# ZechangSun/QFA

Measured on AMD Instinct MI355X. Metric: spectra/sec per EM step, higher is better.
Workload: dtype f32

## Files before the change

### qfa_amd/csrc/qfa_grads_t.h

```cpp
#pragma once
#include "qfa_common.h"
#include "qfa_xdl_kernels.h"
#include "qfa_gt_layout.h"

struct GtPlan {
    int T16, PB, R, gpr;
    int nxcd;
    __host__ __device__ int per_xcd() const { return (PB * R + nxcd - 1) / nxcd; }
    __host__ __device__ int items() const { return nxcd * per_xcd(); }
};

template <int KP>
__device__ __forceinline__ void prep_pgt_body(int bid, const float *__restrict__ F, const float *__restrict__ Psi,
                                              const float *__restrict__ omega, const ZPSrc &ZP, int Npix, int Nb, int Nh,
                                              unsigned char *__restrict__ PGT) {
    using GT = GTT<KP>;
    unsigned char *tile = PGT + (size_t)bid * GT::TILE_B;
    const int p0 = GT::PXW * (bid / GT::TPW) + bid % GT::TPW;
    auto pixel = [&](int lo) { return p0 + GT::TPW * lo; };
    __shared__ float f[16][KP + 1];
    __shared__ float tsc[16][3];
    for (int i = threadIdx.x; i < 16 * KP; i += 256) {
        const int px = i / KP, a = i % KP;
        f[px][a] = (pixel(px) < Npix && a < Nh) ? F[(size_t)pixel(px) * Nh + a] : 0.f;
    }
    __syncthreads();
    if (threadIdx.x < 16) {
        float mx = 0.f;
        for (int a = 0; a < KP; ++a) mx = fmaxf(mx, fabsf(f[threadIdx.x][a]));
        int e = 7;
        if (mx > 0.f && mx < 3.0e38f) (void)frexpf(mx, &e);
        e = e < -50 ? -50 : (e > 60 ? 60 : e);
        tsc[threadIdx.x][0] = ldexpf(1.f, 7 - e);
        tsc[threadIdx.x][1] = ldexpf(1.f, 2 * (e - 7));
        tsc[threadIdx.x][2] = ldexpf(1.f, e - 7);
    }
    __syncthreads();
    for (int i = threadIdx.x; i < GT::NKQ * 64; i += 256) {
        const int lane = i & 63, ks = i >> 6;
        const int px = lane & 15, g = lane >> 4;
        const float t1 = tsc[px][0], t2 = t1 * t1;
        float v[8];
#pragma unroll
        for (int j = 0; j < 8; ++j) {
            const int q = 32 * ks + 8 * g + j;
            float x = 0.f;
            if (q < GT::KK2) {
                int a = 0;
                while (a + 1 < KP && pair_index(a + 1, a + 1, KP) <= q) ++a;
                const int b = a + (q - pair_index(a, a, KP));
                x = f[px][a] * f[px][b] * t2;
            } else {
                const int a = q - (32 * (GT::NKQ - 1) + GT::YOFF);
                if (a >= 0 && a < KP) x = f[px][a] * t1;
            }
            v[j] = x;
        }
        unsigned char *dst = tile + ks * GT::BLK_B + lane * 16;
        u32x4 ph, pm;
        split8h(v, ph, pm);
        *reinterpret_cast<u32x4 *>(dst) = ph;
        *reinterpret_cast<u32x4 *>(dst + 1024) = pm;
    }
    if (threadIdx.x < 128) {
        const int j = threadIdx.x, px = pixel(j & 15);
        float v = 0.f;
        if (j < 16) v = px < Npix ? Psi[px] : 0.f;
        else if (j < 32) v = px < Nb ? omega[px] : 0.f;
        else if (j < 80 && ZP.on() && px < Nb) {
            const float4 q = ZP.at(px);
            v = j < 48 ? q.x : (j < 64 ? q.y : q.z);
        } else if (j >= GT::PAR_IT2 && j < GT::PAR_SBETA) v = tsc[j & 15][j < GT::PAR_IT1 ? 1 : 2];
        else if (j >= GT::PAR_SBETA) v = f16_weight_scale(px < Npix ? Psi[px] : 1.f);
        reinterpret_cast<float *>(tile + GT::OFF_PAR)[j] = v;
    }
    float *fr = reinterpret_cast<float *>(tile + GT::OFF_F);
    for (int i = threadIdx.x; i < 16 * KP; i += 256) fr[i] = f[i / KP][i % KP];
}

#ifndef QFA_GT_STAMPS
#define QFA_GT_STAMPS 0
#endif
#if QFA_GT_STAMPS
__device__ unsigned long long qfa_gt_stamps[2 * 16];
#define GTS(i)                                                                                 \
    {                                                                                          \
        __builtin_amdgcn_sched_barrier(0);                                                     \
        unsigned long long t_;                                                                 \
        asm volatile("s_memtime %0\n\ts_waitcnt lgkmcnt(0)" : "=s"(t_)::"memory");             \
        st_[i] += (unsigned)(t_ - st_last);                                                    \
        st_last = t_;                                                                          \
        __builtin_amdgcn_sched_barrier(0);                                                     \
    }
#else
#define GTS(i) {}
#endif
template <int KP, bool HASA, bool ZF, bool IDX, bool EXACT>
__global__ __launch_bounds__(512, 2) void k_grads_t(qfa_params_t p, qfa_batch_t bt, qfa_tau_t tau, int B, int Npix, int Nb,
                                                    int Nh, GtPlan gp, const unsigned char *__restrict__ PGT,
                                                    const unsigned char *__restrict__ PST, const float4 *__restrict__ ZS,
                                                    float *__restrict__ accum,
                                                    float *__restrict__ slab, double *__restrict__ slabS, int slab_stride,
                                                    Scal64 *__restrict__ sc64) {
    using GT = GTT<KP>;
    __shared__ __attribute__((aligned(16))) unsigned char lds[GT::L_TOTAL];
    const int tid = threadIdx.x;
    const int lane = tid & 63;
    const int wv8 = wave_uniform(tid >> 6);
    const int lo = lane & 15, g = lane >> 4;
    const int item = ((int)blockIdx.x % gp.nxcd) * gp.per_xcd() + ((int)blockIdx.x / gp.nxcd);
    const bool idle = item >= gp.PB * gp.R;
    const int rr = idle ? 0 : item / gp.PB, pb = idle ? 0 : item % gp.PB;
    const int G = (B + 15) >> 4;
    const int g0 = rr * gp.gpr;
    const int n = idle ? 0 : max(0, min(gp.gpr, G - g0));
    constexpr int TPW = GT::TPW, PXW = GT::PXW;
    const int wt = pb + gp.PB * wv8;
#ifndef QFA_GT_ONLY
#define QFA_GT_ONLY 0
#endif
    const bool active = !idle && wt < gp.T16 && (QFA_GT_ONLY == 0 || (QFA_GT_ONLY == 1) == (wv8 < 4));
    int px[TPW];
    bool inb[TPW], blue[TPW];
#pragma unroll
    for (int j = 0; j < TPW; ++j) {
        px[j] = PXW * wt + TPW * lo + j;
        inb[j] = active && px[j] < Npix;
        blue[j] = active && px[j] < Nb;
    }
    const bool blueTile = active && PXW * wt < Nb;
    const DevConsts k = load_consts(p, tau);
    const bool det = slab != nullptr;
    float *accF = det ? slab + (size_t)rr * (size_t)slab_stride : accum;
    float *accA = accF + (size_t)Npix * Nh;
    float *accS = accum + (size_t)Npix * Nh + 3 * (size_t)Npix + Nb;

#if QFA_GT_STAMPS
    unsigned st_[8];
    for (int i = 0; i < 8; ++i) st_[i] = 0;
    unsigned long long st_last;
    asm volatile("s_memtime %0\n\ts_waitcnt lgkmcnt(0)" : "=s"(st_last)::"memory");
#endif
    const unsigned char *tile[TPW];
    u32x4 IBh[TPW][GT::NKQ], IBm[TPW][GT::NKQ];
    float Psi[TPW], om[TPW], ti[TPW], pwi[TPW], l2i[TPW], offl[TPW];
    float it2[TPW], it1[TPW];
    float sbeta[TPW];
    f32x4 zfac = {1.f, 1.f, 1.f, 1.f};
#pragma unroll
    for (int j = 0; j < TPW; ++j) {
        tile[j] = PGT + (size_t)(active ? TPW * wt + j : 0) * GT::TILE_B;
#pragma unroll
        for (int ks = 0; ks < GT::NKQ; ++ks) {
            IBh[j][ks] = *reinterpret_cast<const u32x4 *>(tile[j] + ks * GT::BLK_B + lane * 16);
            IBm[j][ks] = *reinterpret_cast<const u32x4 *>(tile[j] + ks * GT::BLK_B + 1024 + lane * 16);
        }
        const float *par = reinterpret_cast<const float *>(tile[j] + GT::OFF_PAR);
        Psi[j] = par[lo]; om[j] = par[16 + lo];
        it2[j] = par[GT::PAR_IT2 + lo]; it1[j] = par[GT::PAR_IT1 + lo];
        sbeta[j] = par[GT::PAR_SBETA + lo];
        ti[j] = ZF ? par[32 + lo] : 0.f; pwi[j] = ZF ? par[48 + lo] : 0.f; l2i[j] = ZF ? par[64 + lo] : 0.f;
        offl[j] = blue[j] ? k.offp : 0.f;
    }

#pragma unroll
    for (int j = 0; j < TPW; ++j) {
#pragma unroll
        for (int ks = 0; ks < GT::NKQ; ++ks) {
            asm volatile("" ::"v"(IBh[j][ks]), "v"(IBm[j][ks]));
        }
        asm volatile("" ::"v"(Psi[j]), "v"(om[j]), "v"(ti[j]), "v"(pwi[j]), "v"(l2i[j]), "v"(it2[j]), "v"(it1[j]), "v"(sbeta[j]));
    }
    asm volatile("" ::"v"(k.tau0), "v"(k.c0), "v"(k.beta), "v"(k.t_amp), "v"(k.t_lscale), "v"(k.t_expo), "v"(k.t_off), "v"(k.offp),
                 "v"(k.k1), "v"(k.omc0));

    f32x4 W[TPW][GT::NWT], gacc[TPW];
    float gPsi[TPW], gOm[TPW], sA[TPW];
    int cnt[TPW];
    f32x4 betaR[TPW], gamR[TPW];
#pragma unroll
    for (int j = 0; j < TPW; ++j) {
#pragma unroll
        for (int a = 0; a < GT::NWT; ++a) W[j][a] = f32x4{0.f, 0.f, 0.f, 0.f};
        gacc[j] = betaR[j] = gamR[j] = f32x4{0.f, 0.f, 0.f, 0.f};
        gPsi[j] = gOm[j] = sA[j] = 0.f;
        cnt[j] = 0;
    }
    double d_tau0 = 0.0, d_c0 = 0.0, d_beta = 0.0;

    unsigned char *stg = lds + GT::L_STG + wv8 * 2 * GT::STG_B;
    const bool fastp = active && PXW * wt + PXW - 1 < Npix;
    const bool zblue = !ZF && blueTile;
    const bool fastz = !zblue || PXW * wt + PXW - 1 < Nb;
    const bool slow = active && !fastp;
    const bool zstrad = active && fastp && !fastz;
    const bool zfb = ZF && blueTile;
    auto mask_start = [&](int h, int pc) __attribute__((always_inline)) {
        const int st = PXW * wt + 16 * h + 4 * pc;
        return slow ? max(0, min(st, Npix - 4)) : st;
    };
    const unsigned RS = (unsigned)bt.row_stride;
    constexpr bool idx = IDX;
    auto row_index = [&](int t, int bufi, unsigned row, auto first_tag) __attribute__((always_inline)) -> unsigned {
        constexpr bool FIRST = decltype(first_tag)::value;
        const unsigned s0 = 16u * (unsigned)(g0 + t);
        if (!idx) return s0 + row;
        if (FIRST || QFA_TRACKED_LOADS) return (unsigned)bt.rows[s0 + row];
        return (unsigned)reinterpret_cast<const int *>(stg + bufi * GT::STG_B + GT::STG_ROWS)[row];
    };
    struct RowIdx {
        unsigned r[TPW], m;
    };
    auto read_rows = [&](int t, int bufi, auto first_tag) __attribute__((always_inline)) {
        RowIdx ri;
        const int last_row = min(15, B - 1 - 16 * (g0 + t));
        auto slot_row = [&](int q) __attribute__((always_inline)) { return (unsigned)min(q ^ ((q >> 2) & 1), last_row); };
        ri.m = row_index(t, bufi, slot_row(lane >> 2), first_tag);
        if constexpr (TPW == 1) ri.r[0] = ri.m;
        else {
#pragma unroll
            for (int i = 0; i < TPW; ++i) ri.r[i] = row_index(t, bufi, slot_row((64 / (4 * TPW)) * i + lane / (4 * TPW)), first_tag);
        }
        return ri;
    };
    constexpr bool RUNP = !IDX && TPW == 1 && !QFA_TRACKED_LOADS;
    struct SpecRun {
        const unsigned char *d, *e, *z, *m;
    } sr{nullptr, nullptr, nullptr, nullptr};
    unsigned sr_vo = 0u, sr_vz = 0u, sr_om = 0u;
    const bool runok = RUNP && active && !slow && !zstrad;
    if (RUNP) {
        const size_t r2 = (size_t)16 * (size_t)(g0 + 2);
        const unsigned q = (unsigned)lane >> 2, row = q ^ ((q >> 2) & 1u), pc = 16u * (unsigned)wt + 4u * ((unsigned)lane & 3u);
        sr.d = uniform_ptr(reinterpret_cast<const unsigned char *>(bt.delta + r2 * RS));
        sr.e = uniform_ptr(reinterpret_cast<const unsigned char *>(bt.error + r2 * RS) - GT::STG_ARR);
        sr.m = uniform_ptr(reinterpret_cast<const unsigned char *>(bt.mask + r2 * RS) - GT::STG_MASK);
        sr.z = zblue ? uniform_ptr(reinterpret_cast<const unsigned char *>(bt.zabs + r2 * (size_t)Nb) - 2 * GT::STG_ARR)
                     : (zfb ? uniform_ptr(reinterpret_cast<const unsigned char *>(ZS + r2) - 2 * GT::STG_ARR) : sr.d);
        sr_om = row * RS + pc;
        sr_vo = 4u * sr_om;
        sr_vz = zblue ? 4u * (row * (unsigned)Nb + pc) : 16u * ((unsigned)lane & 15u);
    }
    auto stage_req = [&](int bufi, int k) __attribute__((always_inline)) {
        if (k == 0) {
            const unsigned dst = wave_uniform(lds_addr(stg + bufi * GT::STG_B));
            asm volatile("s_mov_b32 m0, %2\n\ts_nop 0\n\tglobal_load_lds_dwordx4 %0, %1" ::"v"(sr_vo), "s"(sr.d), "s"(dst) : "memory");
        } else if (k == 1) asm volatile("global_load_lds_dwordx4 %0, %1 offset:1024" ::"v"(sr_vo), "s"(sr.e) : "memory");
        else if (k == 2) asm volatile("global_load_lds_dwordx4 %0, %1 offset:2048" ::"v"(sr_vz), "s"(sr.z) : "memory");
        else asm volatile("global_load_lds_dword %0, %1 offset:3072" ::"v"(sr_om), "s"(sr.m) : "memory");
    };
    const size_t sr_zinc = zblue ? (size_t)64 * (size_t)(unsigned)Nb : (zfb ? (size_t)256 : (size_t)0);
    auto advance_run = [&]() __attribute__((always_inline)) {
        if (!RUNP) return;
        sr.d += (size_t)64 * RS;
        sr.e += (size_t)64 * RS;
        sr.m += (size_t)16 * RS;
        sr.z += sr_zinc;
    };
    auto stage_spectra = [&](int t, int bufi, const RowIdx &ri, auto first_tag) __attribute__((always_inline)) {
        if (!active) return;
        const int s0 = 16 * (g0 + t);
        const int last_row = min(15, B - 1 - s0);
        const unsigned dst = wave_uniform(lds_addr(stg + bufi * GT::STG_B));
        auto slot_row = [&](int q) __attribute__((always_inline)) { return (unsigned)min(q ^ ((q >> 2) & 1), last_row); };
        auto Rof = [&](unsigned row) __attribute__((always_inline)) -> unsigned { return row_index(t, bufi, row, first_tag); };
#if QFA_TRACKED_LOADS
        {
            float *sf = reinterpret_cast<float *>(stg + bufi * GT::STG_B);
            unsigned char *mb = stg + bufi * GT::STG_B + GT::STG_MASK;
#pragma unroll
            for (int i = 0; i < 4 * TPW; ++i) {
                const int e = 64 * i + lane, q = e / PXW, pl = e % PXW;
                const unsigned R = Rof(slot_row(q));
                const int pxx = PXW * wt + pl;
                const unsigned long long o = (unsigned long long)R * RS + (unsigned)min(pxx, Npix - 1);
                sf[0 * (GT::STG_ARR / 4) + q * PXW + pl] = bt.delta[o];
                sf[1 * (GT::STG_ARR / 4) + q * PXW + pl] = bt.error[o];
                if (zblue) sf[2 * (GT::STG_ARR / 4) + q * PXW + pl] = bt.zabs[(unsigned long long)R * (unsigned)Nb + (unsigned)min(pxx, Nb - 1)];
                mb[(pl >> 4) * 256 + q * 16 + (pl & 15)] = pxx < Npix ? bt.mask[o] : (unsigned char)0;
            }
            if (zfb && lane < 16) reinterpret_cast<float4 *>(sf + 2 * (GT::STG_ARR / 4))[lane] = ZS[s0 + min(lane, last_row)];
            (void)dst;
            return;
        }
#endif
        [&]() __attribute__((always_inline)) {
        const unsigned Rm = ri.m;
        if constexpr (!IDX) {
            if (!slow && !zstrad) {
                const float *dbase = uniform_ptr(bt.delta + (size_t)s0 * RS);
                const float *ebase = uniform_ptr(bt.error + (size_t)s0 * RS);
                const uint8_t *mbase = uniform_ptr(bt.mask + (size_t)s0 * RS);
                const float *zbase = zblue ? uniform_ptr(bt.zabs + (size_t)s0 * Nb) : dbase;
                if (zfb && lane < 16) glds16a(uniform_ptr(ZS + s0), 16u * (unsigned)min(lane, last_row), dst + 2 * GT::STG_ARR);
                if constexpr (TPW == 1) {
                    const unsigned row = slot_row(lane >> 2);
                    const unsigned pc = 16u * (unsigned)wt + 4u * (unsigned)(lane & 3);
                    const unsigned o = row * RS + pc;
                    const unsigned vo = 4u * o, vz = 4u * (row * (unsigned)Nb + pc);
                    const unsigned char *eb = reinterpret_cast<const unsigned char *>(ebase) - GT::STG_ARR;
                    const unsigned char *zb = reinterpret_cast<const unsigned char *>(zbase) - 2 * GT::STG_ARR;
                    const unsigned char *mb_ = reinterpret_cast<const unsigned char *>(mbase) - GT::STG_MASK;
                    if (zblue)
                        asm volatile("s_mov_b32 m0, %7\n\ts_nop 0\n\tglobal_load_lds_dwordx4 %0, %3\n\t"
                                     "global_load_lds_dwordx4 %0, %4 offset:1024\n\tglobal_load_lds_dwordx4 %1, %5 offset:2048\n\t"
                                     "global_load_lds_dword %2, %6 offset:3072"
                                     ::"v"(vo), "v"(vz), "v"(o), "s"(dbase), "s"(eb), "s"(zb), "s"(mb_), "s"(dst) : "memory");
                    else
                        asm volatile("s_mov_b32 m0, %5\n\ts_nop 0\n\tglobal_load_lds_dwordx4 %0, %2\n\t"
                                     "global_load_lds_dwordx4 %0, %3 offset:1024\n\tglobal_load_lds_dword %1, %4 offset:3072"
                                     ::"v"(vo), "v"(o), "s"(dbase), "s"(eb), "s"(mb_), "s"(dst) : "memory");
                } else {
                    constexpr int LPR = 4 * TPW, SPI = 64 / LPR;
#pragma unroll
                    for (int h = 0; h < TPW; ++h)
                        glds4a(mbase, slot_row(lane >> 2) * RS + (unsigned)mask_start(h, lane & 3), dst + GT::STG_MASK + h * 256);
#pragma unroll
                    for (int i = 0; i < TPW; ++i) {
                        const unsigned row = slot_row(SPI * i + lane / LPR);
                        const unsigned pc = (unsigned)(PXW * wt) + 4u * (unsigned)(lane % LPR);
                        glds16a(dbase, 4u * (row * RS + pc), dst + i * 1024);
                        glds16a(ebase, 4u * (row * RS + pc), dst + GT::STG_ARR + i * 1024);
                        if (zblue) glds16a(zbase, 4u * (row * (unsigned)Nb + pc), dst + 2 * GT::STG_ARR + i * 1024);
                    }
                }
                return;
            }
        }
        if (!slow) {
            if constexpr (TPW == 1) {
                const unsigned R = ri.r[0];
                unsigned pc = 16u * (unsigned)wt + 4u * (unsigned)(lane & 3);
                asm volatile("" : "+v"(pc));
                const unsigned long long o = (unsigned long long)R * RS + pc;
                if (zfb && lane < 16) glds16a(uniform_ptr(ZS + s0), 16u * (unsigned)min(lane, last_row), dst + 2 * GT::STG_ARR);
                if (zstrad) {
#pragma unroll 1
                    for (int i = 0; i < 4; ++i) {
                        int pz = min(16 * wt + lo, Nb - 1);
                        asm volatile("" : "+v"(pz));
                        glds4p(lane_ptr<2>(bt.zabs, (unsigned long long)Rof(slot_row(4 * i + g)) * (unsigned)Nb + (unsigned)pz), dst + 2 * GT::STG_ARR + i * 256);
                    }
                }
                const unsigned char *pd = lane_ptr<2>(bt.delta, o);
                const unsigned char *pe = lane_ptr<2>(reinterpret_cast<const unsigned char *>(bt.error) - GT::STG_ARR, o);
                const unsigned char *pm = lane_ptr<0>(bt.mask - GT::STG_MASK, o);
                if (zblue && !zstrad) {
                    const unsigned char *pz = lane_ptr<2>(reinterpret_cast<const unsigned char *>(bt.zabs) - 2 * GT::STG_ARR, (unsigned long long)R * (unsigned)Nb + pc);
                    asm volatile("s_mov_b32 m0, %4\n\ts_nop 0\n\tglobal_load_lds_dwordx4 %0, off\n\t"
                                 "global_load_lds_dwordx4 %1, off offset:1024\n\tglobal_load_lds_dwordx4 %2, off offset:2048\n\t"
                                 "global_load_lds_dword %3, off offset:3072"
                                 ::"v"(pd), "v"(pe), "v"(pz), "v"(pm), "s"(dst) : "memory");
                } else
                    asm volatile("s_mov_b32 m0, %3\n\ts_nop 0\n\tglobal_load_lds_dwordx4 %0, off\n\t"
                                 "global_load_lds_dwordx4 %1, off offset:1024\n\tglobal_load_lds_dword %2, off offset:3072"
                                 ::"v"(pd), "v"(pe), "v"(pm), "s"(dst) : "memory");
            } else {
                constexpr int LPR = 4 * TPW;
                if (zfb && lane < 16) glds16a(uniform_ptr(ZS + s0), 16u * (unsigned)min(lane, last_row), dst + 2 * GT::STG_ARR);
#pragma unroll
                for (int h = 0; h < TPW; ++h) {
                    unsigned ms = (unsigned)mask_start(h, lane & 3);
                    asm volatile("" : "+v"(ms));
                    glds4p(lane_ptr<0>(bt.mask, (unsigned long long)Rm * RS + ms), dst + GT::STG_MASK + h * 256);
                }
#pragma unroll
                for (int i = 0; i < TPW; ++i) {
                    unsigned pc = (unsigned)(PXW * wt) + 4u * (unsigned)(lane % LPR);
                    asm volatile("" : "+v"(pc));
                    const unsigned long long o = (unsigned long long)ri.r[i] * RS + pc;
                    glds16p(lane_ptr<2>(bt.delta, o), dst + i * 1024);
                    glds16p(lane_ptr<2>(bt.error, o), dst + GT::STG_ARR + i * 1024);
                    if (zblue && !zstrad) glds16p(lane_ptr<2>(bt.zabs, (unsigned long long)ri.r[i] * (unsigned)Nb + pc), dst + 2 * GT::STG_ARR + i * 1024);
                }
                if (zstrad) {
#pragma unroll 1
                    for (int i = 0; i < 4 * TPW; ++i) {
                        const int e = 64 * i + lane;
                        int pz = min(PXW * wt + e % PXW, Nb - 1);
                        asm volatile("" : "+v"(pz));
                        glds4p(lane_ptr<2>(bt.zabs, (unsigned long long)Rof(slot_row(e / PXW)) * (unsigned)Nb + (unsigned)pz), dst + 2 * GT::STG_ARR + i * 256);
                    }
                }
            }
            return;
        }
        if (zfb && lane < 16) glds16a(uniform_ptr(ZS + s0), 16u * (unsigned)min(lane, last_row), dst + 2 * GT::STG_ARR);
#pragma unroll 1
        for (int h = 0; h < TPW; ++h) {
            unsigned ms = (unsigned)mask_start(h, lane & 3);
            asm volatile("" : "+v"(ms));
            glds4p(lane_ptr<0>(bt.mask, (unsigned long long)Rm * RS + ms), dst + GT::STG_MASK + h * 256);
        }
#pragma unroll 1
        for (int i = 0; i < 4 * TPW; ++i) {
            const int e = 64 * i + lane, pl = e % PXW;
            const unsigned R = Rof(slot_row(e / PXW));
            int pxx = PXW * wt + pl;
            asm volatile("" : "+v"(pxx));
            const unsigned long long o = (unsigned long long)R * RS + (unsigned)min(pxx, Npix - 1);
            glds4p(lane_ptr<2>(bt.delta, o), dst + i * 256);
            glds4p(lane_ptr<2>(bt.error, o), dst + GT::STG_ARR + i * 256);
            if (zblue) glds4p(lane_ptr<2>(bt.zabs, (unsigned long long)R * (unsigned)Nb + (unsigned)min(pxx, Nb - 1)), dst + 2 * GT::STG_ARR + i * 256);
        }
        }();
        if (idx) {
            const int t2 = min(t + 2, n - 1), s2 = 16 * (g0 + t2);
            if (lane < 16) glds4a(uniform_ptr(bt.rows + s2), 4u * (unsigned)min(lane, B - 1 - s2), dst + GT::STG_ROWS);
        }
    };
    int mask_pos[TPW];
#pragma unroll
    for (int j = 0; j < TPW; ++j) {
        const int pl = TPW * lo + j, h = pl >> 4, pi = pl & 15;
        mask_pos[j] = h * 256 + ((slow && !QFA_TRACKED_LOADS) ? 4 * (pi >> 2) + min(3, PXW * wt + pl - mask_start(h, pi >> 2)) : pi);
    }

    int nduty = 0, drank = 0;
    bool duty = true;
    {
        int nd = 0, rk = 0;
#pragma unroll
        for (int w = 0; w < GT::NW; ++w) {
            const int tw = pb + gp.PB * w;
            const bool d = !(tw < gp.T16 && PXW * tw < Nb);
            if (w < wv8 && d) ++rk;
            if (d) ++nd;
        }
        if (nd >= 5) { nduty = nd; drank = rk; duty = !blueTile; }
        else { nduty = GT::NW; drank = wv8; duty = true; }
    }
    const int s1_q = GT::S1_PCS / nduty, s1_r = GT::S1_PCS % nduty, z_q = GT::Z_PCS / nduty, z_r = GT::Z_PCS % nduty;
    const int s1_first = drank * s1_q + min(drank, s1_r), z_first = drank * z_q + min(drank, z_r);
    const int s1_req = duty ? s1_q + (drank < s1_r ? 1 : 0) : 0, z_req = duty ? z_q + (drank < z_r ? 1 : 0) : 0;
    auto issue_S1 = [&](int t) __attribute__((always_inline)) {
        const unsigned char *src = uniform_ptr(PST + (size_t)(g0 + t) * GT::STATE_B + s1_first * 1024);
        const unsigned dst = wave_uniform(lds_addr(lds + GT::L_S1 + (t & 1) * GT::S1P_B + s1_first * 1024));
        for (int j = 0; j < s1_req; ++j) glds16a(src + 1024 * j, (unsigned)lane * 16u, dst + 1024 * j);
    };
    auto issue_Z = [&](int t) __attribute__((always_inline)) {
        const unsigned char *src = uniform_ptr(PST + (size_t)(g0 + t) * GT::STATE_B + GT::S1P_B + z_first * 1024);
        const unsigned dst = wave_uniform(lds_addr(lds + GT::L_Z + (t & 1) * GT::ZP_B + z_first * 1024));
        for (int j = 0; j < z_req; ++j) glds16a(src + 1024 * j, (unsigned)lane * 16u, dst + 1024 * j);
    };

    struct Part {
        const unsigned char *src;
        unsigned dst;
        int cnt;
    };
    struct NoPart {};
    constexpr unsigned PBIAS = QFA_TRACKED_LOADS ? 0u : 4096u;
    const unsigned lane16 = (unsigned)lane * 16u;
    auto part_begin = [&](const auto &pt) __attribute__((always_inline)) {
        if constexpr (std::is_same_v<std::decay_t<decltype(pt)>, Part>) {
#if !QFA_TRACKED_LOADS
            asm volatile("s_mov_b32 m0, %0\n\ts_nop 0" ::"s"(pt.dst));
#endif
        }
    };
    auto piece = [&](const auto &pt, int j) __attribute__((always_inline)) {
        if constexpr (std::is_same_v<std::decay_t<decltype(pt)>, Part>) {
            if (j < pt.cnt) {
#if QFA_TRACKED_LOADS
                glds16a(pt.src + 1024 * j, lane16, pt.dst + 1024 * j);
#else
#define QFA_PC(J) case J: asm volatile("global_load_lds_dwordx4 %0, %1 offset:%2" ::"v"(lane16), "s"(pt.src), "n"(1024 * J - 4096)); break;
                switch (j) { QFA_PC(0) QFA_PC(1) QFA_PC(2) QFA_PC(3) QFA_PC(4) QFA_PC(5) QFA_PC(6) QFA_PC(7) default: break; }
#undef QFA_PC
#endif
            }
        }
    };
    static_assert((GT::Z_PCS + 4) / 5 <= 8 && (GT::S1_PCS + 4) / 5 <= 8, "a wave's run of a part: at most eight pieces (immediate offsets)");

    f32x4 afy[TPW], aq[TPW];
#pragma unroll
    for (int j = 0; j < TPW; ++j) afy[j] = aq[j] = f32x4{0.f, 0.f, 0.f, 0.f};
    auto stage1 = [&](int t, const auto &pt) __attribute__((always_inline)) {
        __builtin_amdgcn_s_setprio(2);
        part_begin(pt);
        const unsigned char *sp = lds + GT::L_S1 + (t & 1) * GT::S1P_B + lane * 16;
#pragma unroll
        for (int j = 0; j < TPW; ++j) afy[j] = aq[j] = f32x4{0.f, 0.f, 0.f, 0.f};
        constexpr int NP = GT::S1NP;
        u32x4 aop[2][NP];
#pragma unroll
        for (int pc = 0; pc < NP; ++pc) aop[0][pc] = *reinterpret_cast<const u32x4 *>(sp + pc * 1024);
        f32x4 isc[2] = {f32x4{1.f, 1.f, 1.f, 1.f}, f32x4{1.f, 1.f, 1.f, 1.f}};
        const unsigned char *sq = lds + GT::L_S1 + (t & 1) * GT::S1P_B + GT::S1_SCALES + 32 * g;
        isc[0] = *reinterpret_cast<const f32x4 *>(sq);
        isc[1] = *reinterpret_cast<const f32x4 *>(sq + 16);
        zfac = *reinterpret_cast<const f32x4 *>(lds + GT::L_S1 + (t & 1) * GT::S1P_B + GT::S1_ZFAC + 16 * g);
#pragma unroll
        for (int ks = 0; ks < GT::NKS; ++ks) {
            if (ks + 1 < GT::NKS) {
#pragma unroll
                for (int pc = 0; pc < NP; ++pc)
                    aop[(ks + 1) & 1][pc] = *reinterpret_cast<const u32x4 *>(sp + (ks + 1) * GT::BLK_B + pc * 1024);
            }
            piece(pt, ks);
            if (ks == GT::NKS - 1) piece(pt, GT::NKS);
            const u32x4 &ah = aop[ks & 1][0], &am = aop[ks & 1][1];
#pragma unroll
            for (int j = 0; j < TPW; ++j) {
                if (ks < GT::NKQ) aq[j] = xdl3h(ah, am, IBh[j][ks], IBm[j][ks], aq[j]);
                else afy[j] = xdl3h(ah, am, IBh[j][GT::NKQ - 1], IBm[j][GT::NKQ - 1], afy[j]);
            }
        }
#pragma unroll
        for (int j = 0; j < TPW; ++j)
#pragma unroll
            for (int r = 0; r < 4; ++r) {
                aq[j][r] = (aq[j][r] * isc[r >> 1][2 * (r & 1)]) * it2[j];
                afy[j][r] = (afy[j][r] * isc[r >> 1][2 * (r & 1) + 1]) * it1[j];
            }
        GTS(5)
        __builtin_amdgcn_s_setprio(0);
    };
    float dv[TPW][4], sgv[TPW][4], zv[TPW][4];
    unsigned mk[TPW][4];
    RowIdx ri_next{};
#pragma unroll
    for (int j = 0; j < TPW; ++j)
#pragma unroll
        for (int r = 0; r < 4; ++r) { dv[j][r] = sgv[j][r] = zv[j][r] = 0.f; mk[j][r] = 0u; }
    auto take = [&](int t) __attribute__((always_inline)) {
        const unsigned char *sb = stg + (t & 1) * GT::STG_B;
#pragma unroll
        for (int r = 0; r < 4; ++r) {
            const int q = (4 * g + r) ^ (g & 1);
            if constexpr (TPW == 1) {
                dv[0][r] = *reinterpret_cast<const float *>(sb + (q * 16 + lo) * 4);
                sgv[0][r] = *reinterpret_cast<const float *>(sb + GT::STG_ARR + (q * 16 + lo) * 4);
                if (!ZF && blueTile) zv[0][r] = *reinterpret_cast<const float *>(sb + 2 * GT::STG_ARR + (q * 16 + lo) * 4);
            } else {
                typedef float f32x2t __attribute__((ext_vector_type(2)));
                const f32x2t d2 = *reinterpret_cast<const f32x2t *>(sb + (q * PXW + TPW * lo) * 4);
                const f32x2t s2 = *reinterpret_cast<const f32x2t *>(sb + GT::STG_ARR + (q * PXW + TPW * lo) * 4);
                dv[0][r] = d2[0]; dv[TPW - 1][r] = d2[1];
                sgv[0][r] = s2[0]; sgv[TPW - 1][r] = s2[1];
                if (!ZF && blueTile) {
                    const f32x2t z2 = *reinterpret_cast<const f32x2t *>(sb + 2 * GT::STG_ARR + (q * PXW + TPW * lo) * 4);
                    zv[0][r] = z2[0]; zv[TPW - 1][r] = z2[1];
                }
            }
#pragma unroll
            for (int j = 0; j < TPW; ++j) mk[j][r] = sb[GT::STG_MASK + q * 16 + mask_pos[j]];
        }
    };
    auto stage2_t = [&](auto blue_tag, int t, const auto &pt) __attribute__((always_inline)) {
        constexpr bool BLUE = decltype(blue_tag)::value;
        const int s0 = 16 * (g0 + t);
        take(t);
        float zqx[4] = {0.f, 0.f, 0.f, 0.f}, zqy[4] = {0.f, 0.f, 0.f, 0.f}, zqz[4] = {0.f, 0.f, 0.f, 0.f};
        if (ZF && BLUE) {
            const unsigned char *sb = stg + (t & 1) * GT::STG_B;
#pragma unroll
            for (int r = 0; r < 4; ++r) {
                const float4 q = reinterpret_cast<const float4 *>(sb + 2 * GT::STG_ARR)[4 * g + r];
                zqx[r] = q.x; zqy[r] = q.y; zqz[r] = q.z;
            }
        }
        if (IDX && t + 2 < n) ri_next = read_rows(t + 2, t & 1, std::false_type{});
        bool wvm[TPW][4];
        asm volatile("s_waitcnt lgkmcnt(0)" ::: "memory");
#pragma unroll
        for (int j = 0; j < TPW; ++j)
#pragma unroll
            for (int r = 0; r < 4; ++r) asm volatile("" : "+v"(sgv[j][r]), "+v"(mk[j][r]));
        __builtin_amdgcn_sched_barrier(0);
#pragma unroll
        for (int j = 0; j < TPW; ++j)
#pragma unroll
            for (int r = 0; r < 4; ++r) wvm[j][r] = inb[j] & (s0 + 4 * g + r < B) & (mk[j][r] != 0u);
        GTS(6)
        part_begin(pt);
        piece(pt, 0);
        piece(pt, 1);
        __builtin_amdgcn_sched_barrier(0);
        GTS(2)
        float t_tau0 = 0.f, t_c0 = 0.f, t_beta = 0.f;
#pragma unroll
        for (int j = 0; j < TPW; ++j) {
        float e1 = 0.f, e2 = 0.f;
#pragma unroll
        for (int r = 0; r < 4; ++r) {
            const bool wv_ = wvm[j][r];
            const float dd = wv_ ? dv[j][r] : 0.f;
            const float sg = sgv[j][r];
            if (BLUE) {
                float l2 = 0.f, pw, Ab, re, ex;
                if (ZF) {
                    pw = zqy[r] * pwi[j];
                    Ab = fast_exp2(fmaf(zqx[r], ti[j], offl[j]));
                    ex = fast_exp2(k.k1 * pw);
                    re = k.omc0 - ex;
                } else {
                    l2 = fast_log2(1.0f + zv[j][r]);
                    pw = fast_exp2(k.beta * l2);
                    const float tauv = k.t_amp * fast_exp2(k.t_expo * (l2 + k.t_lscale)) + k.t_off;
                    Ab = fast_exp2(-tauv * QFA_LOG2E);
                    ex = fast_exp2(-k.tau0 * pw * QFA_LOG2E);
                    re = 1.0f - k.c0 - ex;
                }
                if (HASA) Ab = bt.A_blue[(size_t)min(s0 + 4 * g + r, B - 1) * Nb + (unsigned)min(px[j], Nb - 1)];
                const float Av = (ZF && !HASA) ? Ab : (blue[j] ? Ab : 1.f);
                const float zd = (ZF && !HASA) ? re * re : (blue[j] ? re * re : 0.f);
                const float A2 = Av * Av;
                const float ozd = om[j] * zd;
                const float D = A2 * Psi[j] + ozd + sg * sg;
                const float wD = wv_ ? fast_rcp(D) : 0.f;
                const float wDA = wD * Av;
                const float uu = wD * (dd - Av * afy[j][r]);
                const float dS = wD - wDA * wDA * aq[j][r];
                const float h = dS - uu * uu;
                gPsi[j] = fmaf(A2, h, gPsi[j]);
                gOm[j] = fmaf(h, zd, gOm[j]);
                const float root = fmaf(-k.tau0, pw, k.omc0);
                const float er = h * ozd * zd * root;
                const float ee = h * om[j] * re;
                const float e = EXACT ? ee : er, et = EXACT ? -ee * ex : er;
                if (ZF) {
                    const float ep = et * zqy[r];
                    e1 += ep;
                    e2 = fmaf(ep, zqz[r], e2);
                } else {
                    t_tau0 -= et * pw;
                    t_beta -= et * (k.tau0 * pw * (l2 * QFA_LN2));
                }
                t_c0 -= e;
                cnt[j] += wv_ ? 1 : 0;
                const float bb = wDA * Av;
                sA[j] += bb * Av;
                betaR[j][r] = bb * (sbeta[j] * zfac[r]);
                gamR[j][r] = Av * uu;
            } else {
                const float D = Psi[j] + sg * sg;
                const float wD = wv_ ? fast_rcp(D) : 0.f;
                const float uu = wD * (dd - afy[j][r]);
                const float dS = wD - wD * wD * aq[j][r];
                gPsi[j] += dS - uu * uu;
                cnt[j] += wv_ ? 1 : 0;
                betaR[j][r] = wD * (sbeta[j] * zfac[r]);
                sA[j] += wD;
                gamR[j][r] = uu;
            }
            if (r & 1) {
                __builtin_amdgcn_sched_barrier(0);
                if (j == TPW - 1) {
                    piece(pt, r == 1 ? 2 : 4);
                    piece(pt, r == 1 ? 3 : 5);
                    if (r == 3) piece(pt, 6);
                }
            }
        }
        if (BLUE && ZF) {
            const float t1 = pwi[j] * e1;
            t_tau0 -= t1;
            t_beta -= k.tau0 * QFA_LN2 * fmaf(pwi[j], e2, l2i[j] * t1);
        }
        }
        if (BLUE) {
            d_tau0 += (double)t_tau0;
            d_c0 += (double)t_c0;
            d_beta += (double)t_beta;
        }
    };
    auto stage2 = [&](int t, const auto &pt) __attribute__((always_inline)) {
        if (blueTile) stage2_t(std::true_type{}, t, pt);
        else stage2_t(std::false_type{}, t, pt);
    };

    const int nfull = max(0, min(n, (B >> 4) - g0));
    auto stage3 = [&](int t, const auto &pt) __attribute__((always_inline)) {
        __builtin_amdgcn_s_setprio(2);
        const bool run = RUNP && runok && t + 2 < nfull;
        if (t + 2 < n && !run) {
            const RowIdx ri = IDX ? ri_next : read_rows(t + 2, t & 1, std::false_type{});
            stage_spectra(t + 2, t & 1, ri, std::false_type{});
        }
        if (!RUNP) part_begin(pt);
        const unsigned char *zp = lds + GT::L_Z + (t & 1) * GT::ZP_B + lane * 16;
        u32x4 bhl[TPW], bmm[TPW], bhh[TPW];
#pragma unroll
        for (int j = 0; j < TPW; ++j) {
            unsigned h01, m01, h23, m23;
            split2h(betaR[j][0], betaR[j][1], h01, m01);
            split2h(betaR[j][2], betaR[j][3], h23, m23);
            bhh[j] = u32x4{h01, h23, h01, h23}; bmm[j] = u32x4{m01, m23, 0u, 0u}; bhl[j] = bhh[j];
        }
        constexpr int ZD = 3 < GT::NWT ? 3 : GT::NWT, ZR = ZD + 1;
        u32x4 zop[ZR][2];
        auto rdz = [&](int a) __attribute__((always_inline)) {
            const unsigned char *q = zp + (a < GT::NWT ? a * GT::ZT_B : GT::Z_B);
            zop[a % ZR][0] = *reinterpret_cast<const u32x4 *>(q);
            if (a == GT::NWT) zop[a % ZR][1] = *reinterpret_cast<const u32x4 *>(q + 1024);
        };
#pragma unroll
        for (int a = 0; a < ZD; ++a) rdz(a);
#pragma unroll
        for (int a = 0; a < GT::NWT; ++a) {
            if (a + ZD <= GT::NWT) rdz(a + ZD);
            __builtin_amdgcn_sched_barrier(0);
            if constexpr (RUNP) {
                constexpr int RQS = 2, P0 = 3 * RQS + 1;
                static_assert(P0 + 7 <= GT::NWT, "piece sites");
                if (a < P0) { if (a % RQS == 0 && run && (a / RQS != 2 || blueTile)) stage_req(t & 1, a / RQS); }
                else {
                    if (a == P0) part_begin(pt);
                    if (a - P0 < 7) piece(pt, a - P0);
                }
            } else if (a % 2 == 0) piece(pt, a / 2);
            const u32x4 &Z1 = zop[a % ZR][0];
#pragma unroll
            for (int j = 0; j < TPW; ++j) {
                W[j][a] = xdlh(Z1, bhh[j], xdlh(Z1, bmm[j], W[j][a]));
            }
            __builtin_amdgcn_sched_barrier(0);
        }
        const u32x4 &P1 = zop[GT::NWT % ZR][0], &P2 = zop[GT::NWT % ZR][1];
#pragma unroll
        for (int j = 0; j < TPW; ++j) {
            unsigned h01, m01, l01, h23, m23, l23;
            split2(gamR[j][0], gamR[j][1], h01, m01, l01);
            split2(gamR[j][2], gamR[j][3], h23, m23, l23);
            const u32x4 ghl = {h01, h23, l01, l23}, gmm = {m01, m23, m01, m23}, ghh = {h01, h23, h01, h23};
            gacc[j] = xdl(P2, ghh, xdl(P2, gmm, xdl(P1, ghl, gacc[j])));
        }
        advance_run();
        __builtin_amdgcn_s_setprio(0);
    };

    if (n > 0) {
        stage_spectra(0, 0, read_rows(0, 0, std::true_type{}), std::true_type{});
        if (n > 1) stage_spectra(1, 1, read_rows(1, 1, std::true_type{}), std::true_type{});
        issue_S1(0);
        if (n > 1) issue_S1(1);
        issue_Z(0);
    }
    dma_wait<0>();
    step_barrier();
    const bool lead = wv8 < 4;
    const NoPart none{};
    if (active && n > 0) {
        stage1(0, none);
        if (lead) stage2(0, none);
    }
    auto walk = [&]() __attribute__((always_inline)) {
        const unsigned char *zsrc = uniform_ptr(PST + (size_t)(g0 + 1) * GT::STATE_B + GT::S1P_B + z_first * 1024 + PBIAS);
        const unsigned char *ssrc = uniform_ptr(PST + (size_t)(g0 + 2) * GT::STATE_B + s1_first * 1024 + PBIAS);
        const unsigned zd0 = wave_uniform(lds_addr(lds + GT::L_Z + z_first * 1024)) + PBIAS;
        const unsigned sd0 = wave_uniform(lds_addr(lds + GT::L_S1 + s1_first * 1024)) + PBIAS;
        unsigned zdst = zd0 + GT::ZP_B, sdst = sd0;
        auto next = [&]() __attribute__((always_inline)) {
            zsrc += GT::STATE_B; ssrc += GT::STATE_B;
            zdst = 2 * zd0 + GT::ZP_B - zdst; sdst = 2 * sd0 + GT::S1P_B - sdst;
        };
        if (lead) {
            for (int t = 0; t < n; ++t) {
                dma_wait<0>();
                GTS(0)
                step_barrier();
                GTS(1)
                const Part pz{zsrc, zdst, t + 1 < n ? z_req : 0}, ps{ssrc, sdst, t + 2 < n ? s1_req : 0};
                stage3(t, pz);
                GTS(4)
                if (t + 1 < n) {
                    stage1(t + 1, ps);
                    stage2(t + 1, none);
                    GTS(3)
                }
                next();
            }
        } else {
            for (int t = 0; t < n; ++t) {
                dma_wait<0>();
                GTS(0)
                step_barrier();
                GTS(1)
                const Part pz{zsrc, zdst, t + 1 < n ? z_req : 0}, ps{ssrc, sdst, t + 2 < n ? s1_req : 0};
                stage2(t, none);
                GTS(3)
                stage3(t, ps);
                GTS(4)
                if (t + 1 < n) stage1(t + 1, pz);
                next();
            }
        }
    };
    auto finish = [&]() __attribute__((always_inline)) {
#if QFA_GT_STAMPS
    if (blockIdx.x == 100 && (wv8 == 0 || wv8 == 4) && lane == 0) {
        st_[7] = n;
        for (int i = 0; i < 8; ++i) qfa_gt_stamps[(wv8 >> 2) * 16 + i] = st_[i];
    }
#endif
    dma_wait<0>();

    if (active) {
#pragma unroll
        for (int j = 0; j < TPW; ++j) {
            const float *fr = reinterpret_cast<const float *>(tile[j] + GT::OFF_F) + lo * KP;
            const float winv = 0.0078125f / sbeta[j];
            f32x4 acc = {0.f, 0.f, 0.f, 0.f};
            if constexpr (GT::APT == 1) {
#pragma unroll
                for (int a4 = 0; a4 < KP / 4; ++a4) {
                    const float4 f4 = *reinterpret_cast<const float4 *>(fr + 4 * a4);
                    const float fa[4] = {f4.x, f4.y, f4.z, f4.w};
#pragma unroll
                    for (int jj = 0; jj < 4; ++jj)
#pragma unroll
                        for (int r = 0; r < 4; ++r) acc[r] = fmaf(fa[jj], W[j][4 * a4 + jj][r], acc[r]);
                }
            } else {
#pragma unroll
                for (int wtile = 0; wtile < GT::NWT; ++wtile) {
                    const float fa = fr[2 * wtile + (g >> 1)];
#pragma unroll
                    for (int r = 0; r < 4; ++r) acc[r] = fmaf(fa, W[j][wtile][r], acc[r]);
                }
#pragma unroll
                for (int r = 0; r < 4; ++r) acc[r] += __shfl_xor(acc[r], 32);
            }
#pragma unroll
            for (int r = 0; r < 4; ++r) acc[r] = fmaf(acc[r], winv, gacc[j][r]);
            if (inb[j] && (GT::APT == 1 || g < 2)) {
#pragma unroll
                for (int r = 0; r < 4; ++r) {
                    const int b = (GT::APT == 1 ? 4 * g : 4 * (g & 1)) + r;
                    if (b < Nh) {
                        float *q = accF + (size_t)px[j] * Nh + b;
                        if (det) *q = acc[r];
                        else atomicAdd(q, acc[r]);
                    }
                }
            }
            float vsA = sA[j], vgPsi = 0.5f * gPsi[j], vgOm = 0.5f * gOm[j], vcnt = (float)cnt[j];
#pragma unroll
            for (int o = 16; o <= 32; o <<= 1) {
                vsA += __shfl_xor(vsA, o);
                vgPsi += __shfl_xor(vgPsi, o);
                vgOm += __shfl_xor(vgOm, o);
                vcnt += __shfl_xor(vcnt, o);
            }
            if (inb[j]) {
                const float v = g == 0 ? vsA : (g == 1 ? vgPsi : (g == 2 ? vgOm : vcnt));
                const bool ok = g != 2 || px[j] < Nb;
                float *q = accA + (g == 0 ? px[j] : (g == 1 ? Npix + px[j] : (g == 2 ? 2 * Npix + px[j] : 2 * Npix + Nb + px[j])));
                if (ok) {
                    if (det) *q = v;
                    else atomicAdd(q, v);
                }
            }
        }
    }
    double s_tau0 = d_tau0, s_c0 = d_c0, s_beta = d_beta;
    for (int o = 32; o >= 1; o >>= 1) {
        s_tau0 += __shfl_xor(s_tau0, o);
        s_c0 += __shfl_xor(s_c0, o);
        s_beta += __shfl_xor(s_beta, o);
    }
    if (det) {
        if (lane == 0) {
            double *q = slabS + ((size_t)blockIdx.x * GT::NW + wv8) * 3;
            q[0] = s_tau0; q[1] = s_c0; q[2] = s_beta;
        }
    } else {
        scal64_commit(sc64, s_tau0, s_c0, s_beta, gridDim.x * (unsigned)GT::NW, accS);
    }
    };
    if (!active) {
        for (int t = 0; t < n; ++t) {
            dma_wait<0>();
            step_barrier();
            if (t + 1 < n) issue_Z(t + 1);
            if (t + 2 < n) issue_S1(t + 2);
        }
    } else walk();
    finish();
}
```

Before: 33.79 million.

## Unroll steady-state pipeline by two with compile-time parity and full-tile specialization

Splits the per-step walk loop into a steady-state section unrolled by two, with buffer parity as a compile-time constant, followed by a generic tail loop. In the steady section, stage2 drops its bounds masks because the tiles are known full, and stage3 skips the runtime staging branch (running-pointer mode or unconditional staging). The piece count gets a compile-time maximum so the switch over load offsets can be pruned. The goal is to remove per-step scalar branching and address arithmetic from the hot loop, at the cost of larger code and more instruction-cache pressure.

```diff
diff --git a/qfa_amd/csrc/qfa_grads_t.h b/qfa_amd/csrc/qfa_grads_t.h
--- a/qfa_amd/csrc/qfa_grads_t.h
+++ b/qfa_amd/csrc/qfa_grads_t.h
@@ -416,6 +416,8 @@
         mask_pos[j] = h * 256 + ((slow && !QFA_TRACKED_LOADS) ? 4 * (pi >> 2) + min(3, PXW * wt + pl - mask_start(h, pi >> 2)) : pi);
     }
 
+    constexpr int MIN_DUTY = 5;
+    static_assert(MIN_DUTY <= GT::NW, "the parts go to MIN_DUTY duty waves or to all NW");
     int nduty = 0, drank = 0;
     bool duty = true;
     {
@@ -427,7 +429,7 @@
             if (w < wv8 && d) ++rk;
             if (d) ++nd;
         }
-        if (nd >= 5) { nduty = nd; drank = rk; duty = !blueTile; }
+        if (nd >= MIN_DUTY) { nduty = nd; drank = rk; duty = !blueTile; }
         else { nduty = GT::NW; drank = wv8; duty = true; }
     }
     const int s1_q = GT::S1_PCS / nduty, s1_r = GT::S1_PCS % nduty, z_q = GT::Z_PCS / nduty, z_r = GT::Z_PCS % nduty;
@@ -449,19 +451,21 @@
         unsigned dst;
         int cnt;
     };
+    struct PartZ : Part { enum { MAX = (GT::Z_PCS + MIN_DUTY - 1) / MIN_DUTY }; };
+    struct PartS : Part { enum { MAX = (GT::S1_PCS + MIN_DUTY - 1) / MIN_DUTY }; };
     struct NoPart {};
     constexpr unsigned PBIAS = QFA_TRACKED_LOADS ? 0u : 4096u;
     const unsigned lane16 = (unsigned)lane * 16u;
     auto part_begin = [&](const auto &pt) __attribute__((always_inline)) {
-        if constexpr (std::is_same_v<std::decay_t<decltype(pt)>, Part>) {
+        if constexpr (std::is_base_of_v<Part, std::decay_t<decltype(pt)>>) {
 #if !QFA_TRACKED_LOADS
             asm volatile("s_mov_b32 m0, %0\n\ts_nop 0" ::"s"(pt.dst));
 #endif
         }
     };
     auto piece = [&](const auto &pt, int j) __attribute__((always_inline)) {
-        if constexpr (std::is_same_v<std::decay_t<decltype(pt)>, Part>) {
-            if (j < pt.cnt) {
+        if constexpr (std::is_base_of_v<Part, std::decay_t<decltype(pt)>>) {
+            if (j < std::decay_t<decltype(pt)>::MAX && j < pt.cnt) {
 #if QFA_TRACKED_LOADS
                 glds16a(pt.src + 1024 * j, lane16, pt.dst + 1024 * j);
 #else
@@ -472,15 +476,15 @@
             }
         }
     };
-    static_assert((GT::Z_PCS + 4) / 5 <= 8 && (GT::S1_PCS + 4) / 5 <= 8, "a wave's run of a part: at most eight pieces (immediate offsets)");
+    static_assert(PartZ::MAX <= 8 && PartS::MAX <= 8, "a wave's run of a part: at most eight pieces (immediate offsets)");
 
     f32x4 afy[TPW], aq[TPW];
 #pragma unroll
     for (int j = 0; j < TPW; ++j) afy[j] = aq[j] = f32x4{0.f, 0.f, 0.f, 0.f};
-    auto stage1 = [&](int t, const auto &pt) __attribute__((always_inline)) {
+    auto stage1 = [&](int par, const auto &pt) __attribute__((always_inline)) {
         __builtin_amdgcn_s_setprio(2);
         part_begin(pt);
-        const unsigned char *sp = lds + GT::L_S1 + (t & 1) * GT::S1P_B + lane * 16;
+        const unsigned char *sp = lds + GT::L_S1 + par * GT::S1P_B + lane * 16;
 #pragma unroll
         for (int j = 0; j < TPW; ++j) afy[j] = aq[j] = f32x4{0.f, 0.f, 0.f, 0.f};
         constexpr int NP = GT::S1NP;
@@ -488,10 +492,10 @@
 #pragma unroll
         for (int pc = 0; pc < NP; ++pc) aop[0][pc] = *reinterpret_cast<const u32x4 *>(sp + pc * 1024);
         f32x4 isc[2] = {f32x4{1.f, 1.f, 1.f, 1.f}, f32x4{1.f, 1.f, 1.f, 1.f}};
-        const unsigned char *sq = lds + GT::L_S1 + (t & 1) * GT::S1P_B + GT::S1_SCALES + 32 * g;
+        const unsigned char *sq = lds + GT::L_S1 + par * GT::S1P_B + GT::S1_SCALES + 32 * g;
         isc[0] = *reinterpret_cast<const f32x4 *>(sq);
         isc[1] = *reinterpret_cast<const f32x4 *>(sq + 16);
-        zfac = *reinterpret_cast<const f32x4 *>(lds + GT::L_S1 + (t & 1) * GT::S1P_B + GT::S1_ZFAC + 16 * g);
+        zfac = *reinterpret_cast<const f32x4 *>(lds + GT::L_S1 + par * GT::S1P_B + GT::S1_ZFAC + 16 * g);
 #pragma unroll
         for (int ks = 0; ks < GT::NKS; ++ks) {
             if (ks + 1 < GT::NKS) {
@@ -525,8 +529,8 @@
     for (int j = 0; j < TPW; ++j)
 #pragma unroll
         for (int r = 0; r < 4; ++r) { dv[j][r] = sgv[j][r] = zv[j][r] = 0.f; mk[j][r] = 0u; }
-    auto take = [&](int t) __attribute__((always_inline)) {
-        const unsigned char *sb = stg + (t & 1) * GT::STG_B;
+    auto take = [&](int par) __attribute__((always_inline)) {
+        const unsigned char *sb = stg + par * GT::STG_B;
 #pragma unroll
         for (int r = 0; r < 4; ++r) {
             const int q = (4 * g + r) ^ (g & 1);
@@ -549,20 +553,21 @@
             for (int j = 0; j < TPW; ++j) mk[j][r] = sb[GT::STG_MASK + q * 16 + mask_pos[j]];
         }
     };
-    auto stage2_t = [&](auto blue_tag, int t, const auto &pt) __attribute__((always_inline)) {
+    auto stage2_t = [&](auto blue_tag, auto full_tag, int t, int par, const auto &pt) __attribute__((always_inline)) {
         constexpr bool BLUE = decltype(blue_tag)::value;
+        constexpr bool FULL = decltype(full_tag)::value;
         const int s0 = 16 * (g0 + t);
-        take(t);
+        take(par);
         float zqx[4] = {0.f, 0.f, 0.f, 0.f}, zqy[4] = {0.f, 0.f, 0.f, 0.f}, zqz[4] = {0.f, 0.f, 0.f, 0.f};
         if (ZF && BLUE) {
-            const unsigned char *sb = stg + (t & 1) * GT::STG_B;
+            const unsigned char *sb = stg + par * GT::STG_B;
 #pragma unroll
             for (int r = 0; r < 4; ++r) {
                 const float4 q = reinterpret_cast<const float4 *>(sb + 2 * GT::STG_ARR)[4 * g + r];
                 zqx[r] = q.x; zqy[r] = q.y; zqz[r] = q.z;
             }
         }
-        if (IDX && t + 2 < n) ri_next = read_rows(t + 2, t & 1, std::false_type{});
+        if (IDX && t + 2 < n) ri_next = read_rows(t + 2, par, std::false_type{});
         bool wvm[TPW][4];
         asm volatile("s_waitcnt lgkmcnt(0)" ::: "memory");
 #pragma unroll
@@ -573,7 +578,7 @@
 #pragma unroll
         for (int j = 0; j < TPW; ++j)
 #pragma unroll
-            for (int r = 0; r < 4; ++r) wvm[j][r] = inb[j] & (s0 + 4 * g + r < B) & (mk[j][r] != 0u);
+            for (int r = 0; r < 4; ++r) wvm[j][r] = FULL ? mk[j][r] != 0u : (inb[j] & (s0 + 4 * g + r < B) & (mk[j][r] != 0u));
         GTS(6)
         part_begin(pt);
         piece(pt, 0);
@@ -667,21 +672,25 @@
             d_beta += (double)t_beta;
         }
     };
-    auto stage2 = [&](int t, const auto &pt) __attribute__((always_inline)) {
-        if (blueTile) stage2_t(std::true_type{}, t, pt);
-        else stage2_t(std::false_type{}, t, pt);
+    auto stage2 = [&](auto full_tag, int t, int par, const auto &pt) __attribute__((always_inline)) {
+        if (blueTile) stage2_t(std::true_type{}, full_tag, t, par, pt);
+        else stage2_t(std::false_type{}, full_tag, t, par, pt);
     };
 
     const int nfull = max(0, min(n, (B >> 4) - g0));
-    auto stage3 = [&](int t, const auto &pt) __attribute__((always_inline)) {
+    auto stage3 = [&](auto mode_tag, int t, int par, const auto &pt) __attribute__((always_inline)) {
+        constexpr int MODE = decltype(mode_tag)::value;
+        static_assert(MODE != 2 || RUNP, "running pointers");
         __builtin_amdgcn_s_setprio(2);
-        const bool run = RUNP && runok && t + 2 < nfull;
-        if (t + 2 < n && !run) {
-            const RowIdx ri = IDX ? ri_next : read_rows(t + 2, t & 1, std::false_type{});
-            stage_spectra(t + 2, t & 1, ri, std::false_type{});
+        const bool run = MODE == 2 || (RUNP && runok && t + 2 < nfull);
+        if constexpr (MODE != 2) {
+            if ((MODE == 1 || t + 2 < n) && !run) {
+                const RowIdx ri = IDX ? ri_next : read_rows(t + 2, par, std::false_type{});
+                stage_spectra(t + 2, par, ri, std::false_type{});
+            }
         }
         if (!RUNP) part_begin(pt);
-        const unsigned char *zp = lds + GT::L_Z + (t & 1) * GT::ZP_B + lane * 16;
+        const unsigned char *zp = lds + GT::L_Z + par * GT::ZP_B + lane * 16;
         u32x4 bhl[TPW], bmm[TPW], bhh[TPW];
 #pragma unroll
         for (int j = 0; j < TPW; ++j) {
@@ -706,7 +715,7 @@
             if constexpr (RUNP) {
                 constexpr int RQS = 2, P0 = 3 * RQS + 1;
                 static_assert(P0 + 7 <= GT::NWT, "piece sites");
-                if (a < P0) { if (a % RQS == 0 && run && (a / RQS != 2 || blueTile)) stage_req(t & 1, a / RQS); }
+                if (a < P0) { if (a % RQS == 0 && run && (a / RQS != 2 || blueTile)) stage_req(par, a / RQS); }
                 else {
                     if (a == P0) part_begin(pt);
                     if (a - P0 < 7) piece(pt, a - P0);
@@ -745,7 +754,7 @@
     const NoPart none{};
     if (active && n > 0) {
         stage1(0, none);
-        if (lead) stage2(0, none);
+        if (lead) stage2(std::false_type{}, 0, 0, none);
     }
     auto walk = [&]() __attribute__((always_inline)) {
         const unsigned char *zsrc = uniform_ptr(PST + (size_t)(g0 + 1) * GT::STATE_B + GT::S1P_B + z_first * 1024 + PBIAS);
@@ -757,34 +766,81 @@
             zsrc += GT::STATE_B; ssrc += GT::STATE_B;
             zdst = 2 * zd0 + GT::ZP_B - zdst; sdst = 2 * sd0 + GT::S1P_B - sdst;
         };
+        constexpr int SMODE = RUNP ? 2 : 1;
+        using SFull = std::integral_constant<bool, RUNP>;
+        using SMode = std::integral_constant<int, SMODE>;
+        const int nst = (RUNP ? (runok ? max(0, nfull - 2) : 0) : max(0, n - 2)) & ~1;
+        const unsigned zdst_s[2] = {zd0 + GT::ZP_B, zd0}, sdst_s[2] = {sd0, sd0 + GT::S1P_B};
+        auto steady_lead = [&](int t, int par) __attribute__((always_inline)) {
+            dma_wait<0>();
+            GTS(0)
+            step_barrier();
+            GTS(1)
+            const PartZ pz{{zsrc, zdst_s[par], z_req}};
+            const PartS ps{{ssrc, sdst_s[par], s1_req}};
+            stage3(SMode{}, t, par, pz);
+            GTS(4)
+            stage1(par ^ 1, ps);
+            stage2(SFull{}, t + 1, par ^ 1, none);
+            GTS(3)
+            zsrc += GT::STATE_B; ssrc += GT::STATE_B;
+        };
+        auto steady_rear = [&](int t, int par) __attribute__((always_inline)) {
+            dma_wait<0>();
+            GTS(0)
+            step_barrier();
+            GTS(1)
+            const PartZ pz{{zsrc, zdst_s[par], z_req}};
+            const PartS ps{{ssrc, sdst_s[par], s1_req}};
+            stage2(SFull{}, t, par, none);
+            GTS(3)
+            stage3(SMode{}, t, par, ps);
+            GTS(4)
+            stage1(par ^ 1, pz);
+            zsrc += GT::STATE_B; ssrc += GT::STATE_B;
+        };
+        using Any = std::false_type;
+        using AnyMode = std::integral_constant<int, 0>;
         if (lead) {
-            for (int t = 0; t < n; ++t) {
+            int t = 0;
+            for (; t < nst; t += 2) {
+                steady_lead(t, 0);
+                steady_lead(t + 1, 1);
+            }
+            for (; t < n; ++t) {
                 dma_wait<0>();
                 GTS(0)
                 step_barrier();
                 GTS(1)
-                const Part pz{zsrc, zdst, t + 1 < n ? z_req : 0}, ps{ssrc, sdst, t + 2 < n ? s1_req : 0};
-                stage3(t, pz);
+                const PartZ pz{{zsrc, zdst, t + 1 < n ? z_req : 0}};
+                const PartS ps{{ssrc, sdst, t + 2 < n ? s1_req : 0}};
+                stage3(AnyMode{}, t, t & 1, pz);
                 GTS(4)
                 if (t + 1 < n) {
-                    stage1(t + 1, ps);
-                    stage2(t + 1, none);
+                    stage1((t + 1) & 1, ps);
+                    stage2(Any{}, t + 1, (t + 1) & 1, none);
                     GTS(3)
                 }
                 next();
             }
         } else {
-            for (int t = 0; t < n; ++t) {
+            int t = 0;
+            for (; t < nst; t += 2) {
+                steady_rear(t, 0);
+                steady_rear(t + 1, 1);
+            }
+            for (; t < n; ++t) {
                 dma_wait<0>();
                 GTS(0)
                 step_barrier();
                 GTS(1)
-                const Part pz{zsrc, zdst, t + 1 < n ? z_req : 0}, ps{ssrc, sdst, t + 2 < n ? s1_req : 0};
-                stage2(t, none);
+                const PartZ pz{{zsrc, zdst, t + 1 < n ? z_req : 0}};
+                const PartS ps{{ssrc, sdst, t + 2 < n ? s1_req : 0}};
+                stage2(Any{}, t, t & 1, none);
                 GTS(3)
-                stage3(t, ps);
+                stage3(AnyMode{}, t, t & 1, ps);
                 GTS(4)
-                if (t + 1 < n) stage1(t + 1, pz);
+                if (t + 1 < n) stage1((t + 1) & 1, pz);
                 next();
             }
         }
```

After: 34.67 million, median of 6. 2.6% higher.
